# mjmj531/isaacgym

Measured on AMD Instinct MI355X. Metric: env-steps/sec at N_envs=16384 (1/2/4/8 GPUs) + achieved HBM GB/s vs roofline, higher is better.
Workload: dtype f32; 1 GPU; humanoid_pingpong 3-actor tilt (HumanoidPingpongTiltG1), num_envs=16384 per GPU, random U(-1,1) actions, 2 physics substeps per step, fused step kernel; variant=TT, kind=step, num_envs_per_gpu=16384, global_envs=16384, horizon_stats_every=32, prewarm_launches=512, full=False, launch=HIP graph of 32 steps, replayed, parallelism=env-shard x1, no data-path collective

## Files before the change

### __graft_entry__.py

```python
import os
import sys

ROOT = os.path.dirname(os.path.abspath(__file__))
if ROOT not in sys.path:
    sys.path.insert(0, ROOT)


def build():
    from isaacgym_amd import _lib
    _lib.build(force=False)
    from oracle import binding as oracle_binding
    oracle_binding.build()
    sys.path.insert(0, os.path.join(ROOT, "tests"))
    import shim_binding
    shim_binding.lib()
    import dr_shim_binding
    dr_shim_binding.lib()
    import urdf_assets
    urdf_assets.build_second_arm_library()
    urdf_assets.build_second_ta_library()
    import isaacgym_amd
    L = _lib.lib()
    from isaacgym_amd import scene
    assert L.ppenv_abi_version() == scene.ABI_VERSION


def smoke():
    import numpy as np
    import torch
    from isaacgym_amd import _lib, scene
    from isaacgym_amd.env import PPEnv
    from oracle import binding as oracle_binding
    sys.path.insert(0, os.path.join(ROOT, "tests"))
    import helpers

    assert torch.cuda.is_available(), "smoke() needs the GPU box"
    _lib.lib()
    n = 256
    cfg = scene.build_config("TT", num_envs=n, seed=1)
    env = PPEnv(scene.build_config("TT", num_envs=n, seed=1), device="cuda:0")
    ora = oracle_binding.OracleEnv(cfg)
    probe = helpers.SensitivityProbe(oracle_binding, cfg)
    oa, ra = helpers.obs_atol(), helpers.reward_atol(cfg)
    rng = np.random.default_rng(0)
    excluded = 0
    for t in range(8):
        a = rng.uniform(-1, 1, (n, 7)).astype(np.float32)
        st = ora.get_state()
        env.set_state(st)
        ora.step(a)
        env.step(torch.from_numpy(a).cuda())
        torch.cuda.synchronize()
        keep = ~probe.sensitive(st, a, ora)
        excluded += int((~keep).sum())
        assert np.array_equal(env.reset_buf.cpu().numpy()[keep], ora.reset_buf[keep])
        helpers.assert_close(env.obs_buf.cpu().numpy()[keep], ora.obs_buf[keep], f"smoke: obs, step {t}", atol=oa)
        helpers.assert_close(env.rew_buf.cpu().numpy()[keep], ora.rew_buf[keep], f"smoke: rew, step {t}", atol=ra)
    assert excluded <= 4, excluded
    assert env.status == 0
    env.close()
    print(f"smoke ok: fused HIP step matches the CPU oracle on {n} envs x 8 steps (rtol 1e-4, the tests' atol; {excluded} env-steps on a switch set aside)")


if __name__ == "__main__":
    build()
    if len(sys.argv) > 1 and sys.argv[1] == "smoke":
        smoke()
```

### isaacgym_amd/csrc/ppenv.hip

```cpp
#include <hip/hip_runtime.h>

#include <algorithm>
#include <cstdio>
#include <cstdlib>
#include <cstring>
#include <new>

using std::min;
using std::max;

#if defined(PP_STAMP)
__device__ unsigned long long pp_stamp_buf[4096 * 32];
#endif
#include "ppenv_device.h"

using namespace pp;

namespace {

constexpr int kBlock = 64;
constexpr int kObsStride = PPENV_NUM_OBS + 1;
constexpr int kMaxSplitSubsteps = 4;

struct DevBuffers {
// ... 273 lines not shown
            for (int d = 0; d < ND; d++) {
                q[d] = b.dof_pos[(size_t)(arm * ND + d) * n + i];
                qd[d] = b.dof_vel[(size_t)(arm * ND + d) * n + i];
                tau[d] = 0.f;
                float act = actions[((size_t)i * A + arm) * ND + d];
                if (DR) { if (dr.act_sigma > 0.f) act += dr.act_sigma * dr_gauss(K.seed, (uint32_t)(K.env_id_offset + i), dr_ep0, dr.key_progress, (uint32_t)(arm * ND + d)); }
                target[d] = pd_target(act, T::drive(d).lower, T::drive(d).upper, K.clip_actions);
            }
        }
        PP_STAMP_AT(1);
        for (int s = 0; s < substeps; s++) {
            if (G) {
                if (s >= 2) PP_AWAIT(&s_bflag, s - 1);
                if (active) {
                    ArmGeom<T::kShapes> gg;
                    GeomVisitor<T> gv(gg);
                    fk_sweep<T>(S, q, qd, js, gv);
                    MovingGeom<T>::each(gg, [&](int k, float& v) { s_geom[s & 1][arm][k][lane] = v; });
                }
                publish(&s_gflag[arm], s + 1);
            }
            if (active) {
                if (!G) {
                    NullVisitor nv;
                    fk_sweep<T>(S, q, qd, js, nv);
                }
                arm_substep<T, DR>(S, js, q, qd, target, K.h, tau, &dr);
#pragma unroll
                for (int d = 0; d < ND; d++) { s_q[s][arm * 2 * ND + d][lane] = q[d]; s_q[s][arm * 2 * ND + ND + d][lane] = qd[d]; }
                if (s + 1 == substeps) {
#pragma unroll
                    for (int d = 0; d < ND; d++) s_tau[arm * ND + d][lane] = tau[d];
                }
            }
            publish(&s_flag[arm], s + 1);
            PP_STAMP_AT(2 + 2 * s);
        }
        BodyState bodies[NB];
        PP_STAMP_AT(5);
        if (arm == 0 && active) {
            V3 sv = serve_on ? mk(b.serve[i], b.serve[(size_t)n + i], b.serve[2 * (size_t)n + i])
                             : serve_velocity(K, (uint32_t)(K.env_id_offset + i), b.episode[i] + 1u);
            s_serve[0][lane] = sv.x; s_serve[1][lane] = sv.y; s_serve[2][lane] = sv.z;
        }
        if (active) {
            ArmGeom<T::kShapes> g;
            BodyVisitor<T, false> bv(g, bodies);
            fk_sweep<T>(S, q, qd, js, bv);
            static_body<false>(S, bodies[0]);
            s_paddle[arm * 3 + 0][lane] = bodies[NB - 1].pos.x; s_paddle[arm * 3 + 1][lane] = bodies[NB - 1].pos.y; s_paddle[arm * 3 + 2][lane] = bodies[NB - 1].pos.z;
        }
        if (!dbg_drop_handoff) publish(&s_flag[arm], substeps + 1);
        if (active) {
            V3 bpos[NB], bvel[NB];
#pragma unroll
            for (int j = 0; j < NB; j++) { bpos[j] = bodies[j].pos; bvel[j] = bodies[j].lin; }
            LdsRowStore store{&s_obs[(arm * kBlock + lane) * kObsStride]};
            NoisyRowStore nstore{&s_obs[(arm * kBlock + lane) * kObsStride], dr.obs_sigma, K.seed, (uint32_t)(K.env_id_offset + i), dr_ep0, dr.key_progress,
                                 16u + (uint32_t)(arm * PPENV_NUM_OBS)};
            if (DR && drt.obs_sigma > 0.f) write_obs_bodies(bpos, bvel, S.hinv, nstore);
            else write_obs_bodies(bpos, bvel, S.hinv, store);
        }
        PP_STAMP_AT(6);
        __builtin_amdgcn_wave_barrier();
        flush_obs_cols<0, 6 * NB>(s_obs, b.obs, arm * kBlock, nvalid, (size_t)base * A + arm, A, lane);
        if (kBallStoresDofs) return;
        PP_AWAIT(&s_flag_ball, 1);
        PP_STAMP_AT(7);
        if (active) {
            const bool rst = s_reset[lane] != 0 && K.rc.variant != PPENV_VARIANT_TN;
#pragma unroll
            for (int d = 0; d < ND; d++) {
                st_state(&b.dof_pos[(size_t)(arm * ND + d) * n + i], rst ? K.init_dof_pos[d] : q[d]);
                st_state(&b.dof_vel[(size_t)(arm * ND + d) * n + i], rst ? K.init_dof_vel[d] : qd[d]);
                st_state(&b.dof_force[(size_t)(arm * ND + d) * n + i], tau[d]);
            }
        }
        return;
    }

    PP_STAMP_AT(16);
    constexpr int EB = kBlock / BW;
    const int bw = wave - A;
    const int env = bw * EB + lane;
    const int bi = base + env;
    const bool bactive = lane < EB && bi < n;
    EnvStateT<A> st;
    float rew[A], pre_vx = 0.f;
    long long reset = 0;
    V3 next_serve = mk(0, 0, 0);
    ArmGeom<T::kShapes> g[A];
    V3 bound[A];
    float qs[A * ND], qds[A * ND];
    EnvDR bdr;
    uint32_t bdr_ep0 = 0;
#pragma unroll
    for (int a = 0; a < A; a++) rew[a] = 0.f;
    if (bactive) {
        if (!G) {
#pragma unroll
            for (int d = 0; d < A * ND; d++) { qs[d] = b.dof_pos[(size_t)d * n + bi]; qds[d] = b.dof_vel[(size_t)d * n + bi]; }
        }
        float bl[13];
#pragma unroll
        for (int k = 0; k < 13; k++) bl[k] = b.ball[(size_t)k * n + bi];
        st.ball.p = mk(bl[0], bl[1], bl[2]);
#pragma unroll
        for (int k = 0; k < 4; k++) st.ball.quat[k] = bl[3 + k];
        st.ball.v = mk(bl[7], bl[8], bl[9]);
        st.ball.w = mk(bl[10], bl[11], bl[12]);
        st.progress = b.progress[(size_t)bi * A];
#pragma unroll
        for (int a = 0; a < A; a++) st.flags[a] = b.flags[(size_t)a * n + bi];
        st.episode = b.episode[bi];
        pre_vx = st.ball.v.x;
#pragma unroll
        for (int a = 0; a < A; a++) { static_geometry<T>(K.site[a], g[a]); bound[a] = ld3(K.site[a].bound_center); }
        if (DR) {
            bdr.es = drt.es ? drt.es[bi] : 1.f;
            bdr.fs = drt.fs ? drt.fs[bi] : 1.f;
            bdr.obs_sigma = drt.obs_sigma;
            bdr.key_progress = (uint32_t)st.progress;
            bdr_ep0 = st.episode;
        }
    }
    PP_STAMP_AT(17);
    for (int s = 0; s < substeps; s++) {
        if (G) {
#pragma unroll
            for (int a = 0; a < A; a++) PP_AWAIT(&s_gflag[a], s + 1);
        } else if (s > 0) {
#pragma unroll
            for (int a = 0; a < A; a++) PP_AWAIT(&s_flag[a], s);
            if (bactive) {
#pragma unroll
                for (int a = 0; a < A; a++)
#pragma unroll
                    for (int d = 0; d < ND; d++) { qs[a * ND + d] = s_q[s - 1][a * 2 * ND + d][env]; qds[a * ND + d] = s_q[s - 1][a * 2 * ND + ND + d][env]; }
            }
        }
        PP_STAMP_AT(18 + 2 * s);
        if (bactive) {
#pragma unroll
            for (int a = 0; a < A; a++) {
                if (G) {
                    MovingGeom<T>::each(g[a], [&](int k, float& v) { v = s_geom[s & 1][a][k][env]; });
                } else {
                    JointSave js[ND];
                    GeomVisitor<T> gv(g[a]);
                    fk_sweep<T>(K.site[a], &qs[a * ND], &qds[a * ND], js, gv);
                }
            }
            PP_STAMP_AT(25);
            ball_substep<T, A, DR>(K, st.ball, g, bound, &bdr);
        }
        if (G) publish(&s_bflag, s + 1);
        PP_STAMP_AT(19 + 2 * s);
    }
#pragma unroll
    for (int a = 0; a < A; a++) PP_AWAIT(&s_flag[a], substeps + 1);
    if (bactive) {
        BodyState bodies[A * NB];
        LdsRowStore stores[A];
#pragma unroll
        for (int a = 0; a < A; a++) {
#pragma unroll
            for (int d = 0; d < ND; d++) {
                st.q[a * ND + d] = s_q[substeps - 1][a * 2 * ND + d][env];
                st.qd[a * ND + d] = s_q[substeps - 1][a * 2 * ND + ND + d][env];
                st.dof_force[a * ND + d] = s_tau[a * ND + d][env];
            }
            static_body<false>(K.site[a], bodies[a * NB]);
            bodies[a * NB + NB - 1].pos = mk(s_paddle[a * 3 + 0][env], s_paddle[a * 3 + 1][env], s_paddle[a * 3 + 2][env]);
            stores[a].row = &s_obs[(a * kBlock + env) * kObsStride];
        }
        next_serve = mk(s_serve[0][env], s_serve[1][env], s_serve[2][env]);
        if (DR && drt.obs_sigma > 0.f) {
            NoisyRowStore nstores[A];
#pragma unroll
            for (int a = 0; a < A; a++)
                nstores[a] = NoisyRowStore{stores[a].row, bdr.obs_sigma, K.seed, (uint32_t)(K.env_id_offset + bi), bdr_ep0, bdr.key_progress, 16u + (uint32_t)(a * PPENV_NUM_OBS)};
            post_physics_env<A, false>(K, (uint32_t)(K.env_id_offset + bi), st, bodies, pre_vx, &next_serve, rew, reset, nstores);
        } else
            post_physics_env<A, false>(K, (uint32_t)(K.env_id_offset + bi), st, bodies, pre_vx, &next_serve, rew, reset, stores);
        s_reset[env] = (int)reset;
    }
    publish(&s_flag_ball, 1);
    PP_STAMP_AT(22);
    __builtin_amdgcn_wave_barrier();
    PP_STAMP_AT(23);
#pragma unroll
    for (int a = 0; a < A; a++)
        flush_obs_cols<6 * NB, PPENV_NUM_OBS>(s_obs, b.obs, a * kBlock + bw * EB, BW == 1 ? nvalid : max(0, min(EB, nvalid - bw * EB)),
                                              (size_t)(base + bw * EB) * A + a, A, lane);
    if (bactive) {
        if (kBallStoresDofs) {
#pragma unroll
            for (int d = 0; d < A * ND; d++) {
                st_state(&b.dof_pos[(size_t)d * n + bi], st.q[d]);
                st_state(&b.dof_vel[(size_t)d * n + bi], st.qd[d]);
                st_state(&b.dof_force[(size_t)d * n + bi], st.dof_force[d]);
            }
        }
        store_ball(b, n, bi, st.ball);
        store_task<A>(b, n, bi, st, rew, reset);
    }
    PP_STAMP_AT(24);
}

template <class T, int A>
__global__ __launch_bounds__(kBlock) void init_kernel(const StepConsts K, DevBuffers b, int mode, int serve_on) {
    __shared__ float s_obs[A * kBlock * kObsStride];
    const int n = K.num_envs;
    const int base = blockIdx.x * kBlock;
    const int lane = threadIdx.x;
    const int i = base + lane;
    const int nvalid = min(kBlock, n - base);
    if (i < n) {
        EnvStateT<A> st;
        st.episode = mode == 0 ? 0u : b.episode[i] + 1u;
        V3 serve = serve_on ? mk(b.serve[i], b.serve[(size_t)n + i], b.serve[2 * (size_t)n + i])
                            : serve_velocity(K, (uint32_t)(K.env_id_offset + i), st.episode);
        reset_state(K, st, serve, true);
#pragma unroll
        for (int d = 0; d < A * ND; d++) st.dof_force[d] = 0.f;
        st.progress = 0;
        float rew[A];
#pragma unroll
        for (int a = 0; a < A; a++) {
            st.flags[a] = PPENV_FLAG_NO_BOUNCE;
            rew[a] = 0.f;
            BodyState bodies[NB];
            bodies_of_state<T>(K.site[a], &st.q[a * ND], &st.qd[a * ND], bodies);
            V3 bpos[NB], bvel[NB];
#pragma unroll
            for (int j = 0; j < NB; j++) { bpos[j] = bodies[j].pos; bvel[j] = bodies[j].lin; }
            LdsRowStore store{&s_obs[(a * kBlock + lane) * kObsStride]};
            write_obs(bpos, bvel, K.site[a].hinv, &st.q[a * ND], &st.qd[a * ND], st.ball.p, st.ball.v, store);
        }
        store_state<A>(b, n, i, st, rew, 1);
    }
    __syncthreads();
#pragma unroll
    for (int a = 0; a < A; a++)
        flush_obs_cols<0, PPENV_NUM_OBS>(s_obs, b.obs, a * kBlock, nvalid, (size_t)base * A + a, A, lane);
}

template <class T, int A>
__global__ __launch_bounds__(kBlock) void reset_idx_kernel(const StepConsts K, DevBuffers b, const long long* __restrict__ ids, int count, int refresh_obs,
                                                           int serve_on, uint32_t* status) {
    const int t = blockIdx.x * kBlock + threadIdx.x;
    if (t >= count) return;
    const int n = K.num_envs;
    const long long id = ids[t];
    if (id < 0 || id >= n) return;
    const int i = (int)id;
    EnvStateT<A> st;
#pragma unroll
    for (int d = 0; d < A * ND; d++) { st.q[d] = b.dof_pos[(size_t)d * n + i]; st.qd[d] = b.dof_vel[(size_t)d * n + i]; }
    st.episode = b.episode[i] + 1u;
    const V3 serve = serve_on ? mk(b.serve[i], b.serve[(size_t)n + i], b.serve[2 * (size_t)n + i])
                              : serve_velocity(K, (uint32_t)(K.env_id_offset + i), st.episode);
    reset_state(K, st, serve, K.rc.variant != PPENV_VARIANT_TN);
#pragma unroll
    for (int d = 0; d < A * ND; d++) { b.dof_pos[(size_t)d * n + i] = st.q[d]; b.dof_vel[(size_t)d * n + i] = st.qd[d]; }
    store_ball(b, n, i, st.ball);
    b.episode[i] = st.episode;
#pragma unroll
    for (int a = 0; a < A; a++) {
        b.progress[(size_t)i * A + a] = 0;
        b.flags[(size_t)a * n + i] = PPENV_FLAG_NO_BOUNCE;
        if (refresh_obs) {
            BodyState bodies[NB];
            bodies_of_state<T>(K.site[a], &st.q[a * ND], &st.qd[a * ND], bodies);
            V3 bpos[NB], bvel[NB];
#pragma unroll
            for (int j = 0; j < NB; j++) { bpos[j] = bodies[j].pos; bvel[j] = bodies[j].lin; }
            LdsRowStore store{b.obs + ((size_t)i * A + a) * PPENV_NUM_OBS};
            write_obs(bpos, bvel, K.site[a].hinv, &st.q[a * ND], &st.qd[a * ND], st.ball.p, st.ball.v, store);
        }
    }
}

template <class T>
__global__ void pd_targets_kernel(int rows, float clip, const float* __restrict__ actions, float* __restrict__ out) {
    const int t = blockIdx.x * blockDim.x + threadIdx.x;
    if (t >= rows * ND) return;
    const int d = t % ND;
    float lo = 0.f, hi = 0.f;
#pragma unroll
    for (int k = 0; k < ND; k++)
        if (k == d) { lo = T::drive(k).lower; hi = T::drive(k).upper; }
    out[t] = pd_target(actions[t], lo, hi, clip);
}
__global__ void serve_from_draws_kernel(int form, int m, const float* __restrict__ draws, float* __restrict__ out) {
    const int t = blockIdx.x * blockDim.x + threadIdx.x;
    if (t >= m) return;
    const V3 v = serve_from_draws(form, draws[3 * t], draws[3 * t + 1], draws[3 * t + 2]);
    out[3 * t] = v.x; out[3 * t + 1] = v.y; out[3 * t + 2] = v.z;
}

__global__ __launch_bounds__(kBlock) void post_physics_kernel(const StepConsts K, DevBuffers b, const float* __restrict__ rb,
                                                               float* root, float* dofs, const float* __restrict__ dof_force,
                                                               const float* __restrict__ pre_vx, int serve_on) {
    __shared__ float s_obs[kBlock * kObsStride];
    const int n = K.num_envs;
    const int base = blockIdx.x * kBlock;
// ... 656 lines not shown
```

### isaacgym_amd/csrc/ppenv_device.h

```cpp
#pragma once

#include <math.h>
#include <stddef.h>
#include <stdint.h>
#include <string.h>

#include "../../include/ppenv.h"

#if defined(__HIPCC__)
#define PP_HD __host__ __device__ __forceinline__
#else
#define PP_HD inline __attribute__((always_inline))
#endif

#if defined(PP_STAMP) && defined(__HIP_DEVICE_COMPILE__)
#define PP_STAMP_AT(k)                                                                      \
    do {                                                                                    \
        __builtin_amdgcn_sched_barrier(0);                                                  \
        unsigned long long t_;                                                              \
        asm volatile("s_memtime %0\n\ts_waitcnt lgkmcnt(0)" : "=s"(t_) : : "memory");      \
        __builtin_amdgcn_sched_barrier(0);                                                  \
        if ((threadIdx.x & 63) == 0) pp_stamp_buf[blockIdx.x * 32 + (k)] = t_;                      \
    } while (0)
extern __device__ unsigned long long pp_stamp_buf[];
// ... 428 lines not shown
            M3 Dm = from_sym(Dr);
            M3 Bp;
#pragma unroll
            for (int j = 0; j < 3; j++) {
                V3 x = cross(r, col(Dm, j));
                Bp.m[j] = Br.m[j] + x.x; Bp.m[3 + j] = Br.m[3 + j] + x.y; Bp.m[6 + j] = Br.m[6 + j] + x.z;
            }
            V3 wp0 = cross(r, row(Bp, 0)), wp1 = cross(r, row(Bp, 1)), wp2 = cross(r, row(Bp, 2));
            V3 wb0 = cross(r, row(Br, 0)), wb1 = cross(r, row(Br, 1)), wb2 = cross(r, row(Br, 2));
            cA.xx = Ar.xx + wp0.x + wb0.x; cA.yy = Ar.yy + wp1.y + wb1.y; cA.zz = Ar.zz + wp2.z + wb2.z;
            cA.xy = Ar.xy + wp1.x + wb0.y; cA.xz = Ar.xz + wp2.x + wb0.z; cA.yz = Ar.yz + wp2.y + wb1.z;
            cB = Bp; cD = Dr;
            cn = nr + cross(r, fr); cf = fr;
        }
    }
    V3 aw = mk(0, 0, 0);
    V3 av = ld3(S.base_grav);
#pragma unroll
    for (int i = 0; i < ND; i++) {
        const JointKin J = T::kin(i);
        const int ax = T::axis(i);
        M3 E = ax == 0 ? joint_rot<0>(J.origin_rot, js[i].c, js[i].s) : (ax == 1 ? joint_rot<1>(J.origin_rot, js[i].c, js[i].s) : joint_rot<2>(J.origin_rot, js[i].c, js[i].s));
        V3 r = ld3(J.origin_xyz);
        V3 e = unit(ax);
        V3 aw2 = tmul(E, aw) + cross(js[i].w, e) * qd[i];
        V3 av2 = tmul(E, av + cross(aw, r)) + cross(js[i].v, e) * qd[i];
        float a = (js[i].u - dot(js[i].ua, aw2) - dot(js[i].ub, av2)) * js[i].dinv;
        qdd[i] = a;
        if (ax == 0) aw2.x += a; else if (ax == 1) aw2.y += a; else aw2.z += a;
        aw = aw2; av = av2;
    }
}

template <class T, bool DR = false>
PP_HD void arm_substep(const ArmSite& S, JointSave* js, float* q, float* qd, const float* target, float h, float* tau_drive, const EnvDR* dr = nullptr) {
    float tau[ND], arm[ND], qdd[ND];
#pragma unroll
    for (int d = 0; d < ND; d++) {
        const JointDrive J = T::drive(d);
        const float kp = DR ? J.kp * dr->kp[d] : J.kp, kd = DR ? J.kd * dr->kd[d] : J.kd;
        float err = target[d] - q[d];
        tau[d] = fminf(fmaxf(kp * (err - h * qd[d]) - kd * qd[d], -J.effort), J.effort);
        arm[d] = J.armature + h * kd + h * h * kp;
    }
    aba_solve<T, DR>(S, js, qd, tau, arm, qdd, dr);
#pragma unroll
    for (int d = 0; d < ND; d++) {
        const JointDrive J = T::drive(d);
        const float kp = DR ? J.kp * dr->kp[d] : J.kp, kd = DR ? J.kd * dr->kd[d] : J.kd;
        float err = target[d] - q[d];
        float vn = qd[d] + h * qdd[d];
        tau_drive[d] = fminf(fmaxf(kp * (err - h * vn) - kd * vn, -J.effort), J.effort);
        vn = fminf(fmaxf(vn, -J.vel_limit), J.vel_limit);
        float qn = q[d] + h * vn;
        if (qn > J.upper) { qn = J.upper; vn = fminf(vn, 0.f); }
        if (qn < J.lower) { qn = J.lower; vn = fmaxf(vn, 0.f); }
        q[d] = qn; qd[d] = vn;
    }
}

struct Ball { V3 p, v, w; float quat[4]; };

struct BallConsts {
    float contact_offset, bounce_threshold, depen_cap, r;
    float inv_kr;
    float stick_factor;
};

PP_HD void contact_resolve(const BallConsts& k, Ball& b, V3 n, float s, V3 u, float e, float mu) {
    if (!(s < k.contact_offset)) return;
    V3 vrel = b.v + cross(b.w, n * (-k.r)) - u;
    float vn = dot(vrel, n);
    if (vn < 0.f) {
        float e_eff = (-vn > k.bounce_threshold) ? e : 0.f;
        float jn = -(1.f + e_eff) * vn;
        V3 vt = vrel - n * vn;
        float vt2 = dot(vt, vt);
        if (vt2 > 1e-18f) {
            float inv = rsq_fast(vt2);
            V3 dir = vt * inv;
            float jt = fminf(mu * jn, vt2 * inv * k.stick_factor);
            b.v = b.v - dir * jt;
            b.w = b.w + cross(n, dir) * (jt * k.inv_kr);
        }
        b.v = b.v + n * jn;
    }
    if (s < 0.f) b.p = madd(b.p, n, fminf(-s, k.depen_cap));
}
PP_HD float clampf(float x, float lo, float hi) { return fminf(fmaxf(x, lo), hi); }

PP_HD void contact_box(const BallConsts& k, Ball& b, const ppenv_box& box) {
    V3 d = b.p - ld3(box.center);
    V3 h = ld3(box.half);
    float reach = k.r + k.contact_offset;
    if (fabsf(d.x) > h.x + reach || fabsf(d.y) > h.y + reach || fabsf(d.z) > h.z + reach) return;
    V3 q = mk(clampf(d.x, -h.x, h.x), clampf(d.y, -h.y, h.y), clampf(d.z, -h.z, h.z));
    V3 diff = d - q;
    float d2 = dot(diff, diff);
    V3 n;
    float s;
    if (d2 > 1e-24f) { float inv = rsq_fast(d2); n = diff * inv; s = d2 * inv - k.r; }
    else {
        float px = h.x - fabsf(d.x), py = h.y - fabsf(d.y), pz = h.z - fabsf(d.z);
        if (px <= py && px <= pz) { n = mk(d.x >= 0.f ? 1.f : -1.f, 0, 0); s = -px - k.r; }
        else if (py <= pz) { n = mk(0, d.y >= 0.f ? 1.f : -1.f, 0); s = -py - k.r; }
        else { n = mk(0, 0, d.z >= 0.f ? 1.f : -1.f); s = -pz - k.r; }
    }
    contact_resolve(k, b, n, s, mk(0, 0, 0), box.restitution, box.friction);
}
PP_HD void contact_capsule(const BallConsts& k, Ball& b, V3 a, V3 bb, V3 ua, V3 ub, float radius, float e, float mu) {
    V3 ab = bb - a;
    float l2 = dot(ab, ab), t = 0.f;
    if (l2 > 1e-12f) t = clampf(dot(b.p - a, ab) * rcp_fast(l2), 0.f, 1.f);
    V3 cp = madd(a, ab, t);
    V3 diff = b.p - cp;
    float d2 = dot(diff, diff);
    if (d2 > (radius + k.r + k.contact_offset) * (radius + k.r + k.contact_offset)) return;
    float inv = d2 > 1e-24f ? rsq_fast(d2) : 0.f;
    V3 n = d2 > 1e-24f ? diff * inv : mk(0, 0, 1);
    V3 u = madd(ua, ub - ua, t);
    contact_resolve(k, b, n, d2 * inv - radius - k.r, u, e, mu);
}
PP_HD void contact_disc(const BallConsts& k, Ball& b, V3 cc, V3 nn, V3 uc, V3 nd, float R, float tp, float e, float mu) {
    V3 d = b.p - cc;
    float hgt = dot(d, nn);
    V3 radial = d - nn * hgt;
    float rr2 = dot(radial, radial);
    float reach = k.r + k.contact_offset;
    if (fabsf(hgt) > tp + reach || rr2 > (R + reach) * (R + reach)) return;
    float rr = sqrtf(rr2);
    V3 n, closest;
    float s;
    if (fabsf(hgt) < tp && rr < R) {
        float sg = hgt >= 0.f ? 1.f : -1.f;
        n = nn * sg;
        s = -(tp - fabsf(hgt)) - k.r;
        closest = cc + nn * (sg * tp) + radial;
    } else {
        float dh = hgt - clampf(hgt, -tp, tp);
        float er = fmaxf(rr - R, 0.f);
        V3 diff = nn * dh + (er > 0.f ? radial * (er * rcp_fast(rr)) : mk(0, 0, 0));
        closest = b.p - diff;
        float d2 = dh * dh + er * er;
        float inv = d2 > 1e-24f ? rsq_fast(d2) : 0.f;
        n = d2 > 1e-24f ? diff * inv : nn;
        s = d2 * inv - k.r;
    }
    V3 u = uc + cross(cross(nn, nd), closest - cc);
    contact_resolve(k, b, n, s, u, e, mu);
}

PP_HD V3 lerp(V3 a, V3 b, float f) { return madd(a, b - a, f); }

template <class T, int A, bool DR = false>
PP_HD void ball_substep(const StepConsts& K, Ball& b, const ArmGeom<T::kShapes> (&g)[A], const V3 (&bound)[A], const EnvDR* dr = nullptr) {
    const int M = K.ball_substeps;
    const float hb = K.hb, h = K.h;
    BallConsts k;
    k.contact_offset = K.contact_offset;
    k.bounce_threshold = K.bounce_threshold;
    k.depen_cap = K.depen_cap;
    k.r = K.ball_r;
    k.inv_kr = K.inv_kr;
    k.stick_factor = K.stick_factor;
    const float gdv = K.gdv, damp = K.damp;
    const float ground_z = K.ground_z, ground_e = K.ground_e, ground_mu = K.ground_mu;
    const ppenv_box& table = K.table;
    const ppenv_box& net = K.net;
    const ModelPaddle P = T::paddle();
    const float e_cap = K.e_cap;
    const float pad_e = DR ? fminf(K.paddle_e * dr->es, e_cap) : K.paddle_e, pad_mu = DR ? K.paddle_mu * dr->fs : K.paddle_mu;
    const float reach = k.r + k.contact_offset + 1e-4f;
    const float pad_rr = sqrtf(P.radius * P.radius + P.half_thickness * P.half_thickness) + reach;
    const float pad_r2 = pad_rr * pad_rr;
    V3 sc0[A][T::kShapes], svc[A][T::kShapes];
    float sr2[A][T::kShapes];
#pragma unroll
    for (int arm = 0; arm < A; arm++)
#pragma unroll
        for (int s = 0; s < T::kShapes; s++) {
            sc0[arm][s] = (g[arm].a[s] + g[arm].b[s]) * 0.5f;
            svc[arm][s] = (g[arm].va[s] + g[arm].vb[s]) * 0.5f;
            V3 hl = (g[arm].b[s] - g[arm].a[s]) * 0.5f;
            float rr = sqrtf(dot(hl, hl)) + T::shape(s).radius + reach;
            sr2[arm][s] = rr * rr;
        }
    PP_STAMP_AT(26);
    for (int m = 0; m < M; m++) {
        const float t = (float)m * hb;
        PP_STAMP_AT(27 + (m & 3));
        b.v.z += gdv;
        b.w = b.w * damp;
        contact_resolve(k, b, mk(0, 0, 1), b.p.z - ground_z - k.r, mk(0, 0, 0), ground_e, ground_mu);
        contact_box(k, b, table);
        contact_box(k, b, net);
#pragma unroll
        for (int arm = 0; arm < A; arm++) {
            const ArmGeom<T::kShapes>& ga = g[arm];
            V3 db = b.p - bound[arm];
            if (dot(db, db) < K.bound_r2) {
                V3 cc = madd(ga.pc, ga.vpc, t);
                V3 dpc = b.p - cc;
                if (dot(dpc, dpc) < pad_r2) {
                    V3 nn = madd(ga.pn, ga.pnd, t);
                    nn = nn * rsq_fast(dot(nn, nn));
                    contact_disc(k, b, cc, nn, ga.vpc, ga.pnd, P.radius, P.half_thickness, pad_e, pad_mu);
                }
#pragma unroll
                for (int s = 0; s < T::kShapes; s++) {
                    V3 dsc = b.p - madd(sc0[arm][s], svc[arm][s], t);
                    if (dot(dsc, dsc) < sr2[arm][s]) {
                        const float radius = T::shape(s).radius;
                        const float e = DR ? fminf(K.shape_e[s] * dr->es, e_cap) : K.shape_e[s], mu = DR ? K.shape_mu[s] * dr->fs : K.shape_mu[s];
                        if (T::shape_link(s) < 0)
                            contact_capsule(k, b, ga.a[s], ga.b[s], mk(0, 0, 0), mk(0, 0, 0), radius, e, mu);
                        else
                            contact_capsule(k, b, madd(ga.a[s], ga.va[s], t), madd(ga.b[s], ga.vb[s], t), ga.va[s], ga.vb[s], radius, e, mu);
                    }
                }
            }
        }
        b.p = madd(b.p, b.v, hb);
    }
    PP_STAMP_AT(31);
    float wx = b.w.x, wy = b.w.y, wz = b.w.z, x = b.quat[0], y = b.quat[1], z = b.quat[2], w = b.quat[3];
    float kq = 0.5f * h;
    float nx = x + kq * (wx * w + wy * z - wz * y);
    float ny = y + kq * (wy * w + wz * x - wx * z);
    float nz = z + kq * (wz * w + wx * y - wy * x);
    float nw = w + kq * (-wx * x - wy * y - wz * z);
    float inv = rsq_fast(nx * nx + ny * ny + nz * nz + nw * nw);
    b.quat[0] = nx * inv; b.quat[1] = ny * inv; b.quat[2] = nz * inv; b.quat[3] = nw * inv;
}

PP_HD V3 quat_rotate(const float q[4], V3 v) {
    float qw = q[3];
    V3 qv = mk(q[0], q[1], q[2]);
    float s = 2.0f * (qw * qw) - 1.0f;
    V3 cr = cross(qv, v);
    float d = dot(qv, v);
    return mk(v.x * s + cr.x * qw * 2.0f + qv.x * d * 2.0f, v.y * s + cr.y * qw * 2.0f + qv.y * d * 2.0f,
              v.z * s + cr.z * qw * 2.0f + qv.z * d * 2.0f);
}
PP_HD void heading_quat_inv(const float q[4], float out[4]) {
    V3 rd = quat_rotate(q, mk(1, 0, 0));
    float heading = atan2f(rd.y, rd.x);
    float theta = (-heading) / 2.0f;
    float sz = sinf(theta), w = cosf(theta);
    float nrm = fmaxf(sqrtf(sz * sz + w * w), 1e-9f);
    out[0] = 0.f; out[1] = 0.f; out[2] = sz / nrm; out[3] = w / nrm;
}

PP_HD V3 heading_rotate(const float hinv[4], V3 v) {
    float qw = hinv[3], sz = hinv[2];
    float s = 2.0f * (qw * qw) - 1.0f;
    float k = sz * qw * 2.0f;
    return mk(v.x * s - v.y * k, v.y * s + v.x * k, v.z);
}

struct RewardIn {
    float humanoid_x;
    V3 paddle;
    float pre_vx;
    V3 bp;
    float vx;
    float power;
    long long progress;
};

PP_HD float compute_reward(const RewardConsts& c, const RewardIn& in, uint32_t& flags, long long& reset) {
    const float Bx = in.bp.x, By = in.bp.y, Bz = in.bp.z, vx = in.vx, pre_vx = in.pre_vx;
    const float alpha = c.alpha, penalty = c.penalty, threshold = 0.1f;
    const float power_reward = -c.power_coefficient * in.power;
    const int variant = c.variant;
    uint32_t f = flags;
    float reward;
    long long die = 0;
    if (variant == PPENV_VARIANT_T3) {
        V3 dp = in.paddle - in.bp;
        float dist = sqrtf(dp.x * dp.x + dp.y * dp.y + dp.z * dp.z);
        float pos_reward = 1.0f / (1.0f + 1.5f * dist * dist);
        float vel_reward = (pre_vx < 0.f && vx > 0.f) ? alpha * fabsf(vx) : 0.f;
        reward = pos_reward + power_reward + vel_reward;
        bool missed = Bx < in.paddle.x - 1e-3f;
        if (missed) { reward = reward + penalty; die = 1; }
        if (Bz < threshold) die = 1;
    } else if (variant == PPENV_VARIANT_TT || variant == PPENV_VARIANT_T4) {
        V3 dp = in.paddle - in.bp;
        float dist = sqrtf(dp.x * dp.x + dp.y * dp.y + dp.z * dp.z);
        float pos_reward = 1.0f / (1.0f + 1.5f * dist * dist);
        bool cond = pre_vx < 0.f && vx > 0.f;
        float vel_reward = (cond && !(f & PPENV_FLAG_COND_CALC)) ? alpha * fabsf(vx) : 0.f;
        if (cond) f |= PPENV_FLAG_COND_CALC;
        bool missed = Bx < in.humanoid_x - 0.05f;
        reward = missed ? 0.f + penalty : 0.f;
        bool bounce = Bz < 0.83f && vx > 0.f && By < 0.6f && By > -0.6f;
        float hit = 0.f;
        bool early = Bx < 2.44f && bounce;
        if (early && !(f & PPENV_FLAG_REWARD_CALC)) hit = c.not_hit_table_penalty;
        if (early) { f |= PPENV_FLAG_REWARD_CALC; f &= ~PPENV_FLAG_NO_BOUNCE; }
        bool inx = Bx > 2.44f && Bx < 3.1f;
        bool good = inx && bounce && (f & PPENV_FLAG_NO_BOUNCE);
        if (good && !(f & PPENV_FLAG_REWARD_CALC)) hit = c.hit_table_reward;
        if (good) f |= PPENV_FLAG_REWARD_CALC;
        if (Bx >= 3.1f && vx > 0.f && !(f & PPENV_FLAG_REWARD_CALC)) hit = c.not_hit_table_penalty;
        if (Bx >= 3.1f) f |= PPENV_FLAG_REWARD_CALC;
        float net = (Bx > 1.7f && Bx < 1.8f && vx > 0.f && By < 0.4f && By > -0.4f && Bz > 0.98f && Bz < 1.14f) ? 400.f : 0.f;
        reward += (((pos_reward + power_reward) + vel_reward) + hit) + net;
        if (Bz < threshold) die = 1;
    } else {
        bool hit_paddle = pre_vx < 0.f && vx > 1.0f;
        bool missed = (Bx < in.humanoid_x - 0.05f) || (Bx < in.paddle.x - 0.1f);
        reward = (!(f & PPENV_FLAG_MISSED_CALC) && missed) ? 0.f + penalty : 0.f;
        if (missed) f |= PPENV_FLAG_MISSED_CALC;
        float dy = in.paddle.y - By, dz = in.paddle.z - Bz;
        float dist = sqrtf(dy * dy + dz * dz);
        float pos_reward = 0.f;
        if (!(f & PPENV_FLAG_COND_CALC) || (Bx < in.humanoid_x - 0.05f)) pos_reward = 1.0f * expf(-20.0f * dist * dist);
        float vel_reward = (hit_paddle && !(f & PPENV_FLAG_COND_CALC)) ? alpha * fabsf(vx) : 0.f;
        if (hit_paddle) f |= PPENV_FLAG_COND_CALC;
        reward += (pos_reward + power_reward) + vel_reward;
        if (Bz < threshold) reward = -800.f + reward;
    }
    flags = f;
    reset = (in.progress >= (long long)c.max_episode_length - 1) ? 1 : die;
    return reward;
}

PP_HD float compute_reward_side2(const RewardConsts& c, const RewardIn& in, uint32_t& flags, long long& reset) {
    const float Bx = in.bp.x, By = in.bp.y, Bz = in.bp.z, vx = in.vx, pre_vx = in.pre_vx;
    uint32_t f = flags;
    V3 dp = in.paddle - in.bp;
    float dist = sqrtf(dp.x * dp.x + dp.y * dp.y + dp.z * dp.z);
    float pos_reward = 1.0f / (1.0f + 1.5f * dist * dist);
    bool cond = pre_vx > 0.f && vx < 0.f;
    float vel_reward = (cond && !(f & PPENV_FLAG_COND_CALC)) ? c.alpha * fabsf(vx) : 0.f;
    if (cond) f |= PPENV_FLAG_COND_CALC;
    bool missed = Bx > in.humanoid_x + 0.05f;
    float reward = missed ? 0.f + c.penalty : 0.f;
    bool bounce = Bz < 0.83f && vx < 0.f && By < 0.6f && By > -0.6f;
    float hit = 0.f;
    bool early = Bx > 1.06f && bounce;
    if (early && !(f & PPENV_FLAG_REWARD_CALC)) hit = c.not_hit_table_penalty;
    if (early) { f |= PPENV_FLAG_REWARD_CALC; f &= ~PPENV_FLAG_NO_BOUNCE; }
    bool inx = Bx < 1.06f && Bx > 0.4f;
    bool good = inx && bounce && (f & PPENV_FLAG_NO_BOUNCE);
    if (good && !(f & PPENV_FLAG_REWARD_CALC)) hit = c.hit_table_reward;
    if (good) f |= PPENV_FLAG_REWARD_CALC;
    if (Bx <= 0.4f && vx < 0.f && !(f & PPENV_FLAG_REWARD_CALC)) hit = c.not_hit_table_penalty;
    if (Bx <= 0.4f) f |= PPENV_FLAG_REWARD_CALC;
    float net = (Bx > 1.7f && Bx < 1.8f && vx < 0.f && By < 0.4f && By > -0.4f && Bz > 0.98f && Bz < 1.14f) ? 400.f : 0.f;
    float power_reward = -c.power_coefficient * in.power;
    reward += (((pos_reward + power_reward) + vel_reward) + hit) + net;
    flags = f;
    reset = (in.progress >= (long long)c.max_episode_length - 1) ? 1 : (Bz < 0.1f ? 1 : 0);
    return reward;
}

template <int A>
struct EnvStateT {
    float q[A * ND], qd[A * ND], dof_force[A * ND];
    Ball ball;
    long long progress;
    uint32_t flags[A], episode;
};
using EnvState = EnvStateT<1>;

template <class T, int A, bool DR = false>
PP_HD void simulate_env(const StepConsts& K, const float* actions, EnvStateT<A>& st, BodyState* bodies, float& pre_vx, const EnvDR* dr = nullptr, uint32_t gid = 0) {
    float target[A * ND];
#pragma unroll
    for (int d = 0; d < A * ND; d++) {
        float act = actions[d];
        if (DR) { if (dr->act_sigma > 0.f) act += dr->act_sigma * dr_gauss(K.seed, gid, st.episode, dr->key_progress, (uint32_t)d); }
        target[d] = pd_target(act, T::drive(d % ND).lower, T::drive(d % ND).upper, K.clip_actions);
    }
    pre_vx = st.ball.v.x;
    const int substeps = K.substeps;
    const float h = K.h;
    JointSave js[A][ND];
    ArmGeom<T::kShapes> g[A];
    V3 bound[A];
#pragma unroll
    for (int a = 0; a < A; a++) {
        bound[a] = ld3(K.site[a].bound_center);
        static_geometry<T>(K.site[a], g[a]);
// ... 239 lines not shown
```

Measured before the change: 1.398 billion env-steps/s.

## Skip unreachable ball contact tests with wave-uniform conservative reach mask

Before the ball micro-substeps, each wavefront computes a conservative bound on how far the ball can travel and which colliders (ground, table, net, each arm's bound sphere, paddle, capsule shapes) it could possibly reach. Contact checks for unreachable colliders are then skipped uniformly across the wave via ballot. If any contact moves the ball, the mask falls back to checking everything. This is meant to cut divergent per-substep collision work, at the cost of extra ballots, added register pressure from the sweep struct, and reliance on the floating-point reach bounds staying conservative.

```diff
diff --git a/__graft_entry__.py b/__graft_entry__.py
--- a/__graft_entry__.py
+++ b/__graft_entry__.py
@@ -16,6 +16,8 @@
     shim_binding.lib()
     import dr_shim_binding
     dr_shim_binding.lib()
+    import reach_shim_binding
+    reach_shim_binding.lib()
     import urdf_assets
     urdf_assets.build_second_arm_library()
     urdf_assets.build_second_ta_library()
diff --git a/isaacgym_amd/csrc/ppenv.hip b/isaacgym_amd/csrc/ppenv.hip
--- a/isaacgym_amd/csrc/ppenv.hip
+++ b/isaacgym_amd/csrc/ppenv.hip
@@ -449,7 +449,7 @@
                 }
             }
             PP_STAMP_AT(25);
-            ball_substep<T, A, DR>(K, st.ball, g, bound, &bdr);
+            ball_substep_masked<T, A, DR>(K, st.ball, g, bound, &bdr);
         }
         if (G) publish(&s_bflag, s + 1);
         PP_STAMP_AT(19 + 2 * s);
diff --git a/isaacgym_amd/csrc/ppenv_device.h b/isaacgym_amd/csrc/ppenv_device.h
--- a/isaacgym_amd/csrc/ppenv_device.h
+++ b/isaacgym_amd/csrc/ppenv_device.h
@@ -604,6 +604,17 @@
 
 PP_HD V3 lerp(V3 a, V3 b, float f) { return madd(a, b - a, f); }
 
+PP_HD void ball_orientation(Ball& b, float h) {
+    float wx = b.w.x, wy = b.w.y, wz = b.w.z, x = b.quat[0], y = b.quat[1], z = b.quat[2], w = b.quat[3];
+    float kq = 0.5f * h;
+    float nx = x + kq * (wx * w + wy * z - wz * y);
+    float ny = y + kq * (wy * w + wz * x - wx * z);
+    float nz = z + kq * (wz * w + wx * y - wy * x);
+    float nw = w + kq * (-wx * x - wy * y - wz * z);
+    float inv = rsq_fast(nx * nx + ny * ny + nz * nz + nw * nw);
+    b.quat[0] = nx * inv; b.quat[1] = ny * inv; b.quat[2] = nz * inv; b.quat[3] = nw * inv;
+}
+
 template <class T, int A, bool DR = false>
 PP_HD void ball_substep(const StepConsts& K, Ball& b, const ArmGeom<T::kShapes> (&g)[A], const V3 (&bound)[A], const EnvDR* dr = nullptr) {
     const int M = K.ball_substeps;
@@ -675,15 +686,187 @@
         b.p = madd(b.p, b.v, hb);
     }
     PP_STAMP_AT(31);
-    float wx = b.w.x, wy = b.w.y, wz = b.w.z, x = b.quat[0], y = b.quat[1], z = b.quat[2], w = b.quat[3];
-    float kq = 0.5f * h;
-    float nx = x + kq * (wx * w + wy * z - wz * y);
-    float ny = y + kq * (wy * w + wz * x - wx * z);
-    float nz = z + kq * (wz * w + wx * y - wy * x);
-    float nw = w + kq * (-wx * x - wy * y - wz * z);
-    float inv = rsq_fast(nx * nx + ny * ny + nz * nz + nw * nw);
-    b.quat[0] = nx * inv; b.quat[1] = ny * inv; b.quat[2] = nz * inv; b.quat[3] = nw * inv;
-}
+    ball_orientation(b, h);
+}
+
+PP_HD bool wave_any(bool p) {
+#if defined(__HIP_DEVICE_COMPILE__)
+    return __builtin_amdgcn_ballot_w64(p) != 0ull;
+#else
+    return p;
+#endif
+}
+constexpr uint32_t kReachAll = 0xffffffffu, kReachGround = 1u, kReachTable = 2u, kReachNet = 4u;
+template <class T> constexpr uint32_t reach_bound_bit(int arm) { return 1u << (3 + arm * (2 + T::kShapes)); }
+template <class T> constexpr uint32_t reach_paddle_bit(int arm) { return 2u << (3 + arm * (2 + T::kShapes)); }
+template <class T> constexpr uint32_t reach_shape_bit(int arm, int s) { return 4u << (3 + arm * (2 + T::kShapes) + s); }
+template <class T, int A> constexpr int reach_items() { return 3 + A * (2 + T::kShapes); }
+
+template <class T, int A, bool DR = false>
+struct BallSweep {
+    static_assert(reach_items<T, A>() <= 32, "one mask bit per item");
+    BallConsts k;
+    int M;
+    float hb, gdv, damp, ground_z, ground_e, ground_mu, pad_e, pad_mu, e_cap, reach, pad_rr, pad_r2;
+    V3 sc0[A][T::kShapes], svc[A][T::kShapes];
+    float srr[A][T::kShapes], sr2[A][T::kShapes];
+
+    PP_HD void init(const StepConsts& K, const ArmGeom<T::kShapes> (&g)[A], const EnvDR* dr) {
+        M = K.ball_substeps;
+        hb = K.hb;
+        k.contact_offset = K.contact_offset;
+        k.bounce_threshold = K.bounce_threshold;
+        k.depen_cap = K.depen_cap;
+        k.r = K.ball_r;
+        k.inv_kr = K.inv_kr;
+        k.stick_factor = K.stick_factor;
+        gdv = K.gdv; damp = K.damp;
+        ground_z = K.ground_z; ground_e = K.ground_e; ground_mu = K.ground_mu;
+        const ModelPaddle P = T::paddle();
+        e_cap = K.e_cap;
+        pad_e = DR ? fminf(K.paddle_e * dr->es, e_cap) : K.paddle_e; pad_mu = DR ? K.paddle_mu * dr->fs : K.paddle_mu;
+        reach = k.r + k.contact_offset + 1e-4f;
+        pad_rr = sqrtf(P.radius * P.radius + P.half_thickness * P.half_thickness) + reach;
+        pad_r2 = pad_rr * pad_rr;
+#pragma unroll
+        for (int arm = 0; arm < A; arm++)
+#pragma unroll
+            for (int s = 0; s < T::kShapes; s++) {
+                sc0[arm][s] = (g[arm].a[s] + g[arm].b[s]) * 0.5f;
+                svc[arm][s] = (g[arm].va[s] + g[arm].vb[s]) * 0.5f;
+                V3 hl = (g[arm].b[s] - g[arm].a[s]) * 0.5f;
+                float rr = sqrtf(dot(hl, hl)) + T::shape(s).radius + reach;
+                srr[arm][s] = rr;
+                sr2[arm][s] = rr * rr;
+            }
+    }
+
+    PP_HD uint32_t reach_mask(const StepConsts& K, const Ball& b, const ArmGeom<T::kShapes> (&g)[A], const V3 (&bound)[A]) const {
+        const float T_ = (float)M * hb;
+        const float eps = (float)(2 * M + 32) * 1.1920929e-7f;
+        const float grow = 1.f + 3.f * eps;
+        const float mg = 2.f * eps * (fabsf(b.p.x) + fabsf(b.p.y) + fabsf(b.p.z));
+        const float v2 = dot(b.v, b.v);
+        const float R = T_ * ((v2 > 0.f ? v2 * rsq_fast(v2) : 0.f) + (float)M * fabsf(gdv));
+        uint32_t mask = 0u;
+        if (wave_any(!(b.p.z - ground_z > (k.r + k.contact_offset + R) * grow + mg))) mask |= kReachGround;
+        const float box_reach = k.r + k.contact_offset;
+#pragma unroll
+        for (int bx = 0; bx < 2; bx++) {
+            const ppenv_box& box = bx == 0 ? K.table : K.net;
+            V3 d = b.p - ld3(box.center);
+            V3 h = ld3(box.half);
+            const float lx = (h.x + box_reach + R) * grow + mg, ly = (h.y + box_reach + R) * grow + mg, lz = (h.z + box_reach + R) * grow + mg;
+            if (wave_any(!(fabsf(d.x) > lx || fabsf(d.y) > ly || fabsf(d.z) > lz))) mask |= bx == 0 ? kReachTable : kReachNet;
+        }
+        const float bound_r = sqrtf(K.bound_r2);
+#pragma unroll
+        for (int arm = 0; arm < A; arm++) {
+            const ArmGeom<T::kShapes>& ga = g[arm];
+            V3 db = b.p - bound[arm];
+            const float lb = (bound_r + R) * grow + mg;
+            if (!wave_any(!(dot(db, db) > lb * lb))) continue;
+            mask |= reach_bound_bit<T>(arm);
+            V3 dpc = b.p - ga.pc;
+            const float lp = (pad_rr + R + T_ * (fabsf(ga.vpc.x) + fabsf(ga.vpc.y) + fabsf(ga.vpc.z))) * grow + mg;
+            if (wave_any(!(dot(dpc, dpc) > lp * lp))) mask |= reach_paddle_bit<T>(arm);
+#pragma unroll
+            for (int s = 0; s < T::kShapes; s++) {
+                V3 dsc = b.p - sc0[arm][s];
+                const float ls = (srr[arm][s] + R + T_ * (fabsf(svc[arm][s].x) + fabsf(svc[arm][s].y) + fabsf(svc[arm][s].z))) * grow + mg;
+                if (wave_any(!(dot(dsc, dsc) > ls * ls))) mask |= reach_shape_bit<T>(arm, s);
+            }
+        }
+        return mask;
+    }
+
+    template <bool kFallback = true>
+    PP_HD uint32_t micro_step(const StepConsts& K, Ball& b, const ArmGeom<T::kShapes> (&g)[A], const V3 (&bound)[A], const EnvDR* dr, int m, uint32_t mask) const {
+        const float t = (float)m * hb;
+        const ModelPaddle P = T::paddle();
+        b.v.z += gdv;
+        b.w = b.w * damp;
+        const V3 p_in = b.p, v_in = b.v;
+#define PP_REACH_MOVED() do { if (kFallback && mask != kReachAll && wave_any(b.p.x != p_in.x || b.p.y != p_in.y || b.p.z != p_in.z)) mask = kReachAll; } while (0)
+        if (mask & kReachGround) {
+            contact_resolve(k, b, mk(0, 0, 1), b.p.z - ground_z - k.r, mk(0, 0, 0), ground_e, ground_mu);
+            PP_REACH_MOVED();
+        }
+        if (mask & kReachTable) { contact_box(k, b, K.table); PP_REACH_MOVED(); }
+        if (mask & kReachNet) { contact_box(k, b, K.net); PP_REACH_MOVED(); }
+#pragma unroll
+        for (int arm = 0; arm < A; arm++) {
+            if (!(mask & reach_bound_bit<T>(arm))) continue;
+            const ArmGeom<T::kShapes>& ga = g[arm];
+            V3 db = b.p - bound[arm];
+            const bool inb = dot(db, db) < K.bound_r2;
+            if (!wave_any(inb)) continue;
+            if (mask & reach_paddle_bit<T>(arm)) {
+                V3 cc = madd(ga.pc, ga.vpc, t);
+                V3 dpc = b.p - cc;
+                if (inb && dot(dpc, dpc) < pad_r2) {
+                    V3 nn = madd(ga.pn, ga.pnd, t);
+                    nn = nn * rsq_fast(dot(nn, nn));
+                    contact_disc(k, b, cc, nn, ga.vpc, ga.pnd, P.radius, P.half_thickness, pad_e, pad_mu);
+                }
+                PP_REACH_MOVED();
+            }
+#pragma unroll
+            for (int s = 0; s < T::kShapes; s++) {
+                if (!(mask & reach_shape_bit<T>(arm, s))) continue;
+                V3 dsc = b.p - madd(sc0[arm][s], svc[arm][s], t);
+                if (inb && dot(dsc, dsc) < sr2[arm][s]) {
+                    const float radius = T::shape(s).radius;
+                    const float e = DR ? fminf(K.shape_e[s] * dr->es, e_cap) : K.shape_e[s], mu = DR ? K.shape_mu[s] * dr->fs : K.shape_mu[s];
+                    if (T::shape_link(s) < 0)
+                        contact_capsule(k, b, ga.a[s], ga.b[s], mk(0, 0, 0), mk(0, 0, 0), radius, e, mu);
+                    else
+                        contact_capsule(k, b, madd(ga.a[s], ga.va[s], t), madd(ga.b[s], ga.vb[s], t), ga.va[s], ga.vb[s], radius, e, mu);
+                }
+                PP_REACH_MOVED();
+            }
+        }
+#undef PP_REACH_MOVED
+        if (kFallback && mask != kReachAll && wave_any(b.p.x != p_in.x || b.p.y != p_in.y || b.p.z != p_in.z || b.v.x != v_in.x || b.v.y != v_in.y || b.v.z != v_in.z)) mask = kReachAll;
+        b.p = madd(b.p, b.v, hb);
+        return mask;
+    }
+};
+
+template <class T, int A, bool DR = false>
+PP_HD void ball_substep_masked(const StepConsts& K, Ball& b, const ArmGeom<T::kShapes> (&g)[A], const V3 (&bound)[A], const EnvDR* dr = nullptr) {
+    BallSweep<T, A, DR> sw;
+    sw.init(K, g, dr);
+    uint32_t mask = sw.reach_mask(K, b, g, bound);
+    PP_STAMP_AT(26);
+    for (int m = 0; m < sw.M; m++) {
+        PP_STAMP_AT(27 + (m & 3));
+        mask = sw.micro_step(K, b, g, bound, dr, m, mask);
+    }
+    PP_STAMP_AT(31);
+    ball_orientation(b, K.h);
+}
+#if !defined(__HIP_DEVICE_COMPILE__)
+template <class T, int A, bool DR = false>
+inline void ball_substep_masked(const StepConsts& K, int lanes, Ball* b, const ArmGeom<T::kShapes> (*g)[A], const V3 (*bound)[A], const EnvDR* dr = nullptr,
+                                uint32_t* masks = nullptr) {
+    BallSweep<T, A, DR>* sw = new BallSweep<T, A, DR>[lanes];
+    uint32_t mask = 0u;
+    for (int l = 0; l < lanes; l++) {
+        sw[l].init(K, g[l], DR ? &dr[l] : nullptr);
+        mask |= sw[l].reach_mask(K, b[l], g[l], bound[l]);
+    }
+    if (masks) masks[0] = mask;
+    for (int m = 0; m < K.ball_substeps; m++) {
+        uint32_t next = mask;
+        for (int l = 0; l < lanes; l++) next |= sw[l].micro_step(K, b[l], g[l], bound[l], DR ? &dr[l] : nullptr, m, mask);
+        mask = next;
+        if (masks) masks[m + 1] = mask;
+    }
+    for (int l = 0; l < lanes; l++) ball_orientation(b[l], K.h);
+    delete[] sw;
+}
+#endif
 
 PP_HD V3 quat_rotate(const float q[4], V3 v) {
     float qw = q[3];
```

New measurement: 1.102 billion env-steps/s. 0.788x the previous value.
